# therealadityashankar/hey-buddy

Hardware: AMD Instinct MI355X
Metric: audio clips/sec featurized+trained, 1.5 s @16 kHz, 1/2/4/8 GPU (higher is better)
Workload: dtype f32

## Files before the change

### hey-buddy_amd/csrc/hbk_augment_plan.h

```cpp
#pragma once

#include <algorithm>
#include <cmath>
#include <cstdarg>
#include <cstdint>
#include <cstdio>
#include <numeric>
#include <string>
#include <vector>

namespace hbk {
namespace {

constexpr int kPlanOk = 0, kPlanErrArg = -1, kPlanErrUnsupported = -3;

inline std::string strf(const char* fmt, ...) {
  char buf[512];
  va_list ap;
  va_start(ap, fmt);
  vsnprintf(buf, sizeof(buf), fmt, ap);
  va_end(ap);
  return buf;
}

// ... 79 lines not shown
    return kPlanErrUnsupported;
  }
  return kPlanOk;
}

struct PitchLayout {
  int64_t y = 0;
  int64_t taps = 0;
  int64_t yr = 0;
  int64_t sp = 0;
  int64_t key = 0;
  int64_t ord = 0;
  int64_t gord = 0;
  int64_t total = 0;
};

inline PitchLayout pitch_layout(const PitchGeometry& a, int64_t n) {
  PitchLayout w;
  w.y = 0;
  w.taps = up256(n * a.l1 * 4);
  w.yr = w.taps + up256(int64_t(kPsPhaseMax) * kPsTapMax * 4);
  w.sp = w.yr + up256(n * 8);
  w.key = w.sp + up256(n * 8);
  w.ord = w.key + up256(n * 8);
  w.gord = w.ord + up256(n * 4);
  w.total = w.gord + up256(n * 4);
  return w;
}

struct PitchKnobs {
  bool span = true;
  bool pair = true;
  bool resample_valu = false;
};

struct Grid {
  unsigned x = 1, y = 1, block = 0;
};

struct PitchLaunches {
  bool pair = false;
  int groups = 0;
  Grid taps, span, rank_clips, group, rank_groups, vocoder, resample;
  bool resample_mfma = true;
};

inline PitchLaunches pitch_launches(const PitchGeometry& a, int64_t n, const PitchKnobs& k) {
  PitchLaunches p;
  p.pair = k.span && k.pair;
  p.groups = static_cast<int>((n + kPvClips - 1) / kPvClips);
  p.taps = Grid{unsigned((a.nw * kPsTapMax + 255) / 256), 1, 256};
  p.span = Grid{unsigned((n + 3) / 4), 1, 256};
  p.rank_clips = Grid{unsigned((n + 63) / 64), 1, 1024};
  p.group = Grid{unsigned((p.groups + 255) / 256), 1, 256};
  p.rank_groups = Grid{unsigned((p.groups + 63) / 64), 1, 1024};
  p.vocoder = Grid{unsigned(p.groups), 1, unsigned(128 * kPvClips)};
  const int res_frames = (a.L + a.nw - 1) / a.nw;
  p.resample_mfma = !(k.resample_valu || a.nw > 128);
  p.resample = p.resample_mfma ? Grid{unsigned((res_frames + kRsFrames - 1) / kRsFrames), unsigned(n), 256}
                               : Grid{unsigned((res_frames + kPsResFrames - 1) / kPsResFrames), unsigned(n), 128};
  return p;
}

struct BandStopLayout {
  int64_t sums = 0;
  int64_t taps = 0;
// ... 74 lines not shown
```

### hey-buddy_amd/csrc/hbk_clip_ops.hip

```cpp
#include <algorithm>

#include "hbk_aug_dev.h"

namespace hbk {
namespace {

struct TanhArgs {
  const float* x;
  int64_t x_stride;
  float* out;
  int64_t out_stride;
  int64_t n_clips;
  const float* amount;
  const int32_t* idx;
  int64_t n_entries;
  SrcView view;
};

__device__ __forceinline__ unsigned abs_bits(float v, int s) {
  return s < kT ? (__builtin_bit_cast(unsigned, v) & 0x7FFFFFFFu) : 0xFFFFFFFFu;
}

__global__ void __launch_bounds__(kThreads) __attribute__((amdgpu_waves_per_eu(8)))
tanh_distortion_kernel(TanhArgs a) {
  __shared__ unsigned hist[4096];
  __shared__ float red[32];
  __shared__ unsigned pick[2];
  constexpr int kPer = (kT + kThreads - 1) / kThreads;
  const int64_t n_iter = a.idx ? a.n_entries : a.n_clips;
  for (int64_t e = blockIdx.x; e < n_iter; e += gridDim.x) {
    const int64_t clip = a.idx ? a.idx[e] : e;
    const int tid = opaque_tid();
    const float* x = a.x + clip * a.x_stride;
    float* out = a.out + clip * a.out_stride;
    const float amt = a.amount[clip];
    if (amt != amt) {
      if (out != x) copy_clip(x, out, tid);
      continue;
    }
    float xr[kPer];
    const int pre = a.view.pre ? a.view.pre[clip] : -1, len = a.view.pre ? a.view.len[clip] : 0;
    if (pre >= 0) {
      const int n = min(len, kT);
      const float* row = n > 0 ? a.view.src + clip * a.view.stride : x;
      const int t = opaque_tid();
      const int w0 = __builtin_amdgcn_readfirstlane(t & ~63);
#pragma unroll
      for (int u = 0; u < kPer; ++u) xr[u] = load_placed_wave(row, pre, n, w0 + u * kThreads, t & 63);
    } else {
    const int t = opaque_tid();
#pragma unroll
    for (int u = 0; u < kPer; ++u) {
      const int s = t + u * kThreads;
      xr[u] = s < kT ? *reinterpret_cast<const float*>(reinterpret_cast<const char*>(x) + (static_cast<uint32_t>(s) << 2))
                     : 0.f;
    }
    }
    const double pos = (100.0 - 99.0 * static_cast<double>(amt)) / 100.0 * (kT - 1);
    const int lo = min(max(static_cast<int>(floor(pos)), 0), kT - 1);
    const double frac = pos - lo;
    unsigned prefix = 0, mask = 0, rank = static_cast<unsigned>(lo);
#pragma unroll 1
    for (int p = 0; p < 3; ++p) {
      const int shift = p == 0 ? 19 : (p == 1 ? 9 : 0), bins = p == 0 ? 4096 : (p == 1 ? 1024 : 512);
      const int per_lane = bins >> 6;
      for (int i = tid; i < bins; i += kThreads) hist[i] = 0;
      __syncthreads();
      const int t = opaque_tid();
#pragma unroll
      for (int u = 0; u < kPer; ++u) {
        const unsigned b = abs_bits(xr[u], t + u * kThreads);
        if ((b & mask) == prefix && b != 0xFFFFFFFFu) atomicAdd(&hist[(b >> shift) & (bins - 1)], 1u);
      }
      __syncthreads();
      if (tid < 64) {
        unsigned own = 0;
        for (int i = 0; i < per_lane; ++i) own += hist[per_lane * tid + i];
        unsigned inc = own;
#pragma unroll
        for (int d = 1; d < 64; d <<= 1) {
          const unsigned v = __shfl_up(inc, d, 64);
          if (tid >= d) inc += v;
        }
        const unsigned long long hit = __ballot(inc > rank);
        const int l = __ffsll(static_cast<long long>(hit)) - 1;
        if (tid == l) {
          unsigned r = rank - (inc - own), dsel = per_lane * l;
          for (int i = 0; i < per_lane - 1; ++i) {
            const unsigned h = hist[dsel];
            if (r < h) break;
            r -= h;
            ++dsel;
          }
          pick[0] = dsel;
          pick[1] = r;
        }
      }
      __syncthreads();
      prefix |= pick[0] << shift;
      mask |= static_cast<unsigned>(bins - 1) << shift;
      rank = pick[1];
    }
    float cnt = 0.f, mg = __builtin_inff();
    const int t2 = opaque_tid();
#pragma unroll
    for (int u = 0; u < kPer; ++u) {
// ... 278 lines not shown
```

### hey-buddy_amd/csrc/hbk_pitch.hip

```cpp
#include <atomic>
#include <cstdlib>

#include "hbk_augment_plan.h"
#include "hbk_common.h"

namespace hbk {
namespace {

static_assert(kPsTapMax == HBK_PITCH_SHIFT_MAX_TAPS, "the resampler's tap rows");
static_assert(kPlanOk == HBK_OK && kPlanErrArg == HBK_ERR_ARG && kPlanErrUnsupported == HBK_ERR_UNSUPPORTED,
              "the planner's status values");
#ifndef HBK_PV_ABLATE
#define HBK_PV_ABLATE 0
#endif
#ifndef HBK_PV_F32STATE
#define HBK_PV_F32STATE 0
#endif
#ifndef HBK_PV_RESTART
#if HBK_PV_F32STATE
#define HBK_PV_RESTART 128
#else
#define HBK_PV_RESTART 1024
#endif
#endif
constexpr int kPvRestart = HBK_PV_RESTART;
#if HBK_PV_F32STATE
typedef float pv_t;
#else
typedef double pv_t;
#endif

struct PitchArgs {
  const float* x;
  int64_t x_stride;
  const int32_t* idx;
  int n;
  float* out;
  int64_t out_stride;
  int L, f_in, f_out, l1, orig, nw, width, target;
  double rate;
  float* y;
  float* taps;
  int2* yr;
  int span;
  int2* sp;
  uint64_t* key;
  int32_t* ord;
  int32_t* gord;
};

__device__ __forceinline__ int ps_i0(const PitchArgs& a, int t, float& alpha) {
  const float ts = static_cast<float>(static_cast<double>(t) * a.rate);
  const float fl = floorf(ts);
  alpha = ts - fl;
  return static_cast<int>(fl);
}

struct PvClip {
  float d[kPvRows][8];
  float xs[256];
  float gh[2][kPvGh][8];
  int cnt0;
  int lo, hi;
};
struct PvShared {
  cf tw[256];
  double tw64[256][2];
  float4 wt[3][128];
  PvClip c[kPvClips];
};

__device__ __forceinline__ int pv_g(int b) { return (b & 3) ^ ((b & 4) ? 7 : 0); }

template <int kCtrl>
__device__ __forceinline__ float pv_dpp(float v) {
  return __builtin_bit_cast(float, __builtin_amdgcn_update_dpp(0, __builtin_bit_cast(int, v), kCtrl, 0xF, 0xF, true));
}

template <bool kSwap16>
__device__ __forceinline__ float pv_swap_add(float x, float y) {
  if (kSwap16)
// ... 100 lines not shown
    atomicMax(&C.hi, hi);
  }
}

__device__ __forceinline__ void pv_frames_of(const PitchArgs& a, int lo, int hi, int& tb, int& tl) {
  const int jmax = (a.l1 + kPsPad - 1) / kPsHop;
  tb = 0;
  tl = jmax;
  float al;
  if (lo > hi) {
    tl = -1;
    return;
  }
  if (lo > 2 * kPsPad && a.rate < 2.0) {
    const int fz = (lo - kPsPad) / kPsHop - 1;
    int tg = min(static_cast<int>((fz - 2) / a.rate), a.f_out - 1) & ~(kPvGroup - 1);
    while (tg > 0 && ps_i0(a, tg - 1, al) + 2 > fz) tg -= kPvGroup;
    tb = max(tg, 0);
  }
  if (hi < a.L - 1 - 2 * kPsPad) {
    const int fn = min((hi + kPsPad) / kPsHop, a.f_in - 1);
    int t = max(min(a.f_out - 1, static_cast<int>((fn + 1) / a.rate) + 1), 0);
    while (t > 0 && ps_i0(a, t, al) > fn) --t;
    while (t + 1 < a.f_out && ps_i0(a, t + 1, al) <= fn) ++t;
    tl = min(jmax, t + 36);
  }
}

constexpr int kPsQuant = 360;

__global__ void __launch_bounds__(256) ps_span_kernel(PitchArgs a) {
  const int lane = threadIdx.x & 63, e = blockIdx.x * 4 + (threadIdx.x >> 6);
  if (e >= a.n) return;
  const float* xr = a.x + static_cast<int64_t>(a.idx[e]) * a.x_stride;
  constexpr int kChunk = 64 * 8;
  int lo = INT_MAX, hi = -1;
  for (int p0 = 0; p0 < a.L; p0 += kChunk) {
    float v[8];
#pragma unroll
    for (int j = 0; j < 8; ++j) {
      const int p = p0 + 64 * j + lane;
      v[j] = p < a.L ? xr[p] : 0.f;
    }
#pragma unroll
    for (int j = 0; j < 8; ++j)
      if (v[j] != 0.f) {
        lo = min(lo, p0 + 64 * j + lane);
        hi = max(hi, p0 + 64 * j + lane);
      }
    if (__any(hi >= 0)) break;
  }
  for (int o = 32; o >= 1; o >>= 1) {
    lo = min(lo, __shfl_xor(lo, o, 64));
    hi = max(hi, __shfl_xor(hi, o, 64));
  }
  if (hi >= 0) {
    for (int p1 = a.L; p1 > hi + 1; p1 -= kChunk) {
      float v[8];
      int h = -1;
#pragma unroll
      for (int j = 0; j < 8; ++j) {
        const int p = p1 - kChunk + 64 * j + lane;
        v[j] = (p > hi && p < a.L) ? xr[max(p, 0)] : 0.f;
      }
#pragma unroll
      for (int j = 0; j < 8; ++j)
        if (v[j] != 0.f) h = max(h, p1 - kChunk + 64 * j + lane);
      if (__any(h >= 0)) {
        for (int o = 32; o >= 1; o >>= 1) h = max(h, __shfl_xor(h, o, 64));
        hi = h;
        break;
      }
    }
  }
  if (lane == 0) {
    a.sp[e] = int2{lo, hi};
    const uint64_t q = hi < 0 ? 0 : 1 + static_cast<uint64_t>(hi / kPsQuant), f = hi < 0 ? 0 : static_cast<uint64_t>(lo);
    a.key[e] = (q << 40) | (f << 16) | static_cast<uint64_t>(e);
  }
}

__global__ void __launch_bounds__(1024) ps_rank_kernel(const uint64_t* __restrict__ key, int n,
                                                       int32_t* __restrict__ ord) {
  __shared__ int part[16][64];
  const int lane = threadIdx.x & 63, w = threadIdx.x >> 6, i = blockIdx.x * 64 + lane;
  const uint64_t mine = key[min(i, n - 1)];
  const int per = (n + 15) / 16, j0 = min(w * per, n), j1 = min(j0 + per, n);
  int below = 0;
  for (int jb = j0; jb < j1; jb += 64) {
    const uint64_t kl = jb + lane < j1 ? key[jb + lane] : ~uint64_t(0);
#pragma unroll
    for (int q = 0; q < 64; ++q) {
      const uint32_t hi = __builtin_amdgcn_readlane(static_cast<int>(kl >> 32), q);
      const uint32_t lo = __builtin_amdgcn_readlane(static_cast<int>(kl), q);
      below += ((static_cast<uint64_t>(hi) << 32) | lo) < mine;
    }
// ... 528 lines not shown
#pragma unroll
  for (int ft = 0; ft < kRsFrames / 16; ++ft) {
    rs_f4 acc[2] = {{0.f, 0.f, 0.f, 0.f}, {0.f, 0.f, 0.f, 0.f}};
#pragma unroll
    for (int ks = 0; ks < 5; ++ks) {
      const rs_h8 ah = *reinterpret_cast<const rs_h8*>(&wh[16 * ft + n][32 * ks + 8 * kq]);
      const rs_h8 al = *reinterpret_cast<const rs_h8*>(&wl[16 * ft + n][32 * ks + 8 * kq]);
#pragma unroll
      for (int t = 0; t < 2; ++t) {
        acc[t] = __builtin_amdgcn_mfma_f32_16x16x32_f16(ah, bh[t][ks], acc[t], 0, 0, 0);
        acc[t] = __builtin_amdgcn_mfma_f32_16x16x32_f16(ah, bl[t][ks], acc[t], 0, 0, 0);
        acc[t] = __builtin_amdgcn_mfma_f32_16x16x32_f16(al, bh[t][ks], acc[t], 0, 0, 0);
      }
    }
#pragma unroll
    for (int t = 0; t < 2; ++t) {
      const int ph = 16 * (2 * wave + t) + n;
#pragma unroll
      for (int j = 0; j < 4; ++j) {
        const int i = (f0 + 16 * ft + 4 * kq + j) * a.nw + ph;
        if (ph < a.nw && i < a.L) out[i] = i < a.target ? acc[t][j] * unscale : 0.f;
      }
    }
  }
}

PitchKnobs read_pitch_knobs() {
  PitchKnobs k;
  const char* s = getenv("HBK_PS_SPAN");
  k.span = !(s && s[0] == '0');
  s = getenv("HBK_PS_PAIR");
  k.pair = !(s && s[0] == '0');
  k.resample_valu = getenv("HBK_PS_RESAMPLE_VALU") != nullptr;
  return k;
}

int vocoder_lds_opt_in() {
  constexpr int kDevices = 64;
  static std::atomic<bool> done[kDevices];
  int dev = -1;
  HBK_HIP(hipGetDevice(&dev));
  const bool tracked = dev >= 0 && dev < kDevices;
  if (tracked && done[dev].load(std::memory_order_acquire)) return HBK_OK;
  HBK_HIP(hipFuncSetAttribute(reinterpret_cast<const void*>(ps_vocoder_kernel),
                              hipFuncAttributeMaxDynamicSharedMemorySize, int(sizeof(PvShared))));
  if (tracked) done[dev].store(true, std::memory_order_release);
  return HBK_OK;
}

template <typename... Params, typename... Args>
void launch(void (*kernel)(Params...), const Grid& g, size_t lds, hipStream_t st, Args... args) {
  hipLaunchKernelGGL(kernel, dim3(g.x, g.y), dim3(g.block), lds, st, args...);
}

}

#ifdef HBK_PHASE_TIMING
int pv_phase_take(unsigned long long* out) {
  if (hipMemcpyFromSymbol(out, HIP_SYMBOL(g_pv_phase), sizeof(unsigned long long) * 5) != hipSuccess) return -2;
  unsigned long long z[5] = {};
  (void)hipMemcpyToSymbol(HIP_SYMBOL(g_pv_phase), z, sizeof(z));
  return 0;
}
#endif

}

extern "C" {

int64_t hbk_pitch_shift_workspace_size(int64_t n, int64_t T, int32_t sample_rate, int32_t num, int32_t den) {
  hbk::PitchGeometry g;
  std::string err;
  if (n <= 0 || hbk::pitch_geometry(T, sample_rate, num, den, g, err) != HBK_OK) return 0;
  return hbk::pitch_layout(g, n).total;
}

int hbk_pitch_shift(const float* x, int64_t x_stride, int64_t n, const int32_t* idx, int64_t T, int32_t sample_rate,
                    int32_t num, int32_t den, float* out, int64_t out_stride, void* workspace,
                    int64_t workspace_bytes, void* stream) {
  using namespace hbk;
  if (n < 0) return arg_error("negative n");
  if (n == 0) return HBK_OK;
  if (n > 65535) return arg_error("n > 65535 per call");
  if (!x || !idx || !out || !workspace) return arg_error("NULL pointer");
  PitchGeometry g;
  std::string err;
  const int rc = pitch_geometry(T, sample_rate, num, den, g, err);
  if (rc != HBK_OK) {
    set_error("%s", err.c_str());
    return rc;
  }
  if (x_stride < T || out_stride < T) return arg_error("stride < T");
  const PitchLayout off = pitch_layout(g, n);
  if (workspace_bytes < off.total) return arg_error("workspace too small (hbk_pitch_shift_workspace_size)");
  const PitchKnobs knobs = read_pitch_knobs();
  const PitchLaunches L = pitch_launches(g, n, knobs);
  unsigned char* w = static_cast<unsigned char*>(workspace);
  PitchArgs a{};
  a.x = x;
  a.x_stride = x_stride;
  a.idx = idx;
  a.n = static_cast<int>(n);
  a.out = out;
  a.out_stride = out_stride;
  a.L = g.L, a.f_in = g.f_in, a.f_out = g.f_out, a.l1 = g.l1;
  a.orig = g.orig, a.nw = g.nw, a.width = g.width, a.target = g.target;
  a.rate = g.rate;
  a.y = reinterpret_cast<float*>(w + off.y);
  a.taps = reinterpret_cast<float*>(w + off.taps);
  a.yr = reinterpret_cast<int2*>(w + off.yr);
  a.span = knobs.span ? 1 : 0;
  if (L.pair) {
    a.sp = reinterpret_cast<int2*>(w + off.sp);
    a.key = reinterpret_cast<uint64_t*>(w + off.key);
    a.ord = reinterpret_cast<int32_t*>(w + off.ord);
    a.gord = reinterpret_cast<int32_t*>(w + off.gord);
  }
  const int lds_rc = vocoder_lds_opt_in();
  if (lds_rc != HBK_OK) return lds_rc;
  hipStream_t st = as_stream(stream);
  launch(ps_taps_kernel, L.taps, 0, st, a);
  HBK_LAUNCH_CHECK("ps_taps_kernel");
  if (L.pair) {
    launch(ps_span_kernel, L.span, 0, st, a);
    HBK_LAUNCH_CHECK("ps_span_kernel");
    launch(ps_rank_kernel, L.rank_clips, 0, st, static_cast<const uint64_t*>(a.key), a.n, a.ord);
    HBK_LAUNCH_CHECK("ps_rank_kernel");
    launch(ps_group_kernel, L.group, 0, st, a, L.groups);
    HBK_LAUNCH_CHECK("ps_group_kernel");
    launch(ps_rank_kernel, L.rank_groups, 0, st, static_cast<const uint64_t*>(a.key), L.groups, a.gord);
    HBK_LAUNCH_CHECK("ps_rank_kernel");
  }
  launch(ps_vocoder_kernel, L.vocoder, sizeof(PvShared), st, a);
  HBK_LAUNCH_CHECK("ps_vocoder_kernel");
  launch(L.resample_mfma ? ps_resample_mfma_kernel : ps_resample_kernel, L.resample, 0, st, a);
  HBK_LAUNCH_CHECK(L.resample_mfma ? "ps_resample_mfma_kernel" : "ps_resample_kernel");
  return HBK_OK;
}

}
```

### hey-buddy_amd/heybuddy/_native.py

```python
from __future__ import annotations

import ctypes
import os
import threading
from typing import Optional

import torch

__all__ = ["HBKError", "HBKUnavailable", "lib", "check", "stream_ptr", "require_device",
           "LIB_PATH"]

LIB_PATH = os.environ.get(
    "HBK_LIB",
    os.path.join(os.path.dirname(os.path.dirname(os.path.abspath(__file__))), "lib", "libhbk.so"),
)


class HBKError(RuntimeError):
    """A libhbk.so entry point returned a non-zero status."""


class HBKUnavailable(HBKError):
    """libhbk.so (or a HIP device) is not available: the HIP path cannot run."""

# ... 29 lines not shown
                                     ctypes.POINTER(ctypes.c_double),
                                     ctypes.POINTER(ctypes.c_double),
                                     ctypes.POINTER(ctypes.c_int32)]),
    "hbk_embed_workspace_size": (_c_int, [_vp, _c_int64, ctypes.POINTER(_c_int64)]),
    "hbk_embed_clips": (_c_int, [_vp, _vp, _c_int64, _c_int64, _vp, _vp, _c_int64, _vp]),
    "hbk_embed_split_info": (_c_int, [_vp, ctypes.c_int32, ctypes.POINTER(_c_int64)]),
    "hbk_embed_clips_front": (_c_int, [_vp, _vp, _c_int64, _c_int64, ctypes.c_int32, _vp, _vp, _c_int64, _vp]),
    "hbk_embed_clips_back": (_c_int, [_vp, _vp, _c_int64, ctypes.c_int32, _vp, _vp, _c_int64, _vp]),
    "hbk_embed_windows": (_c_int, [_vp, _vp, _c_int64, _vp, _vp, _c_int64, _vp]),
    "hbk_nan_rows_workspace_size": (_c_int64, [_c_int64]),
    "hbk_nan_rows_fix": (_c_int, [_vp, _c_int64, _c_int64, ctypes.c_uint64, _vp, _c_int64, _vp]),
    "hbk_embed_range_status": (_c_int, [_vp, ctypes.POINTER(ctypes.c_int32), ctypes.c_int32, _vp]),
    "hbk_reverb_plan_create": (_c_int, [_c_int64, ctypes.POINTER(_vp)]),
    "hbk_reverb_plan_destroy": (_c_int, [_vp]),
    "hbk_reverb_spectrum": (_c_int, [_vp, _vp, _c_int64, _c_int64, _vp, _vp]),
    "hbk_augment": (_c_int, [_vp, _vp, _c_int64, _c_int64, _vp, _c_int64, _vp, _vp, _vp, _vp, _vp,
                             _vp, _c_int64, _vp]),
    "hbk_colored_noise": (_c_int, [_vp, _vp, _c_int64, _c_int64, _vp, _c_int64, ctypes.c_uint64, _c_int64, _vp,
                                   _vp, _c_float, _vp, _c_int64, _vp, _c_int64, _vp]),
    "hbk_augment_colored": (_c_int, [_vp, _vp, _c_int64, _c_int64, _vp, _c_int64, _vp, _vp, _vp, _vp, _vp,
                                     _vp, _c_int64, ctypes.c_uint64, _c_int64, _vp, _vp, _c_float, _vp, _c_int64,
                                     _vp, _c_int64, _vp, _c_int64, _vp]),
    "hbk_colored_noise_workspace_size": (_c_int64, [_c_int64, _c_int64]),
    "hbk_colored_noise_ws": (_c_int, [_vp, _vp, _c_int64, _c_int64, _vp, _c_int64, ctypes.c_uint64, _c_int64, _vp,
                                      _vp, _c_float, _vp, _c_int64, _vp, _c_int64, _vp, _c_int64, _vp]),
    "hbk_tanh_distortion": (_c_int, [_vp, _c_int64, _c_int64, _vp, _vp, _c_int64, _vp, _c_int64, _vp]),
    "hbk_band_stop_workspace_size": (_c_int64, [_c_int64, ctypes.c_int32, ctypes.c_int32, _vp]),
    "hbk_band_stop": (_c_int, [_vp, _vp, _c_int64, _c_int64, _vp, _vp, ctypes.c_int32, _vp, _vp, _vp, _vp,
                               ctypes.c_int32, _vp, _vp, _vp, _c_int64, _vp, _c_int64, _vp]),
    "hbk_pitch_shift_workspace_size": (_c_int64, [_c_int64, _c_int64, ctypes.c_int32, ctypes.c_int32,
                                                  ctypes.c_int32]),
    "hbk_pitch_shift": (_c_int, [_vp, _c_int64, _c_int64, _vp, _c_int64, ctypes.c_int32, ctypes.c_int32,
                                 ctypes.c_int32, _vp, _c_int64, _vp, _c_int64, _vp]),
    "hbk_seven_band_eq": (_c_int, [_vp, _c_int64, _c_int64, _vp, _vp, _c_int64, _vp, _c_int64, _vp]),
    "hbk_place_clips": (_c_int, [_vp, _c_int64, _c_int64, _vp, _vp, _vp, _c_int64, _c_int64, _vp]),
    "hbk_place_clips_idx": (_c_int, [_vp, _c_int64, _c_int64, _vp, _vp, _vp, _c_int64, _vp, _c_int64, _c_int64,
                                     _vp]),
    "hbk_seven_band_eq_src": (_c_int, [_vp, _c_int64, _c_int64, _vp, _vp, _c_int64, _vp, _c_int64,
                                       _vp, _c_int64, _vp, _vp, _vp]),
    "hbk_tanh_distortion_src": (_c_int, [_vp, _c_int64, _c_int64, _vp, _vp, _c_int64, _vp, _c_int64,
                                         _vp, _c_int64, _vp, _vp, _vp]),
    "hbk_reverb_plan_set_source": (_c_int, [_vp, _vp, _c_int64, _vp, _vp]),
    "hbk_mlp_set_step_scalars": (_c_int, [_vp, _vp]),
    "hbk_mlp_plan_create": (_c_int, [ctypes.c_int32] * 4 + [ctypes.POINTER(_vp)]),
    "hbk_mlp_plan_create_ex": (_c_int, [ctypes.c_int32] * 6 + [ctypes.POINTER(_vp)]),
    "hbk_mlp_act_forward": (_c_int, [_vp, _c_int64, ctypes.c_int32, ctypes.c_int32, ctypes.c_int32, _vp, _vp]),
    "hbk_mlp_act_backward": (_c_int, [_vp, _vp, _c_int64, ctypes.c_int32, ctypes.c_int32, ctypes.c_int32, _vp,
                                      _vp]),
    "hbk_mlp_plan_create_half": (_c_int, [ctypes.c_int32] * 6 + [_vp, ctypes.POINTER(_vp)]),
    "hbk_mlp_half_layout": (_c_int, [_vp, _vp, ctypes.c_int32]),
    "hbk_mlp_plan_destroy": (_c_int, [_vp]),
    "hbk_mlp_layout": (_c_int, [_vp, ctypes.POINTER(_c_int64), _vp, ctypes.c_int32]),
    "hbk_mlp_workspace_size": (_c_int, [_vp, _c_int64, ctypes.POINTER(_c_int64)]),
    "hbk_mlp_forward": (_c_int, [_vp, _vp, _vp, _c_int64, _vp, _vp, _c_float, ctypes.c_uint64,
                                 _vp, _c_int64, _vp]),
    "hbk_mlp_train_fwd_bwd": (_c_int, [_vp, _vp, _vp, _vp, _c_int64, _c_float, _c_float, _c_float,
                                       _c_float, ctypes.c_uint64, _vp, _vp, _vp, _c_int64, _vp]),
    "hbk_mlp_gate_adam": (_c_int, [_vp, _vp, _vp, _vp, _vp, _vp, _vp, _vp, ctypes.c_int32,
                                   _c_float, _c_float, _c_float, _c_float, _vp]),
    "hbk_mlp_fused_supported": (_c_int, [_vp, ctypes.POINTER(ctypes.c_int32)]),
    "hbk_mlp_step_variant": (_c_int, [_vp, _c_int64, _vp, ctypes.POINTER(ctypes.c_int32)]),
    "hbk_mlp_step_plan_info": (_c_int, [_vp, _c_int64, _vp, ctypes.POINTER(ctypes.c_int32), ctypes.c_int32]),
    "hbk_mlp_step_fwd_bwd": (_c_int, [_vp, _vp, _vp, _c_int64, _vp, _c_int64, _vp, _c_int64, _vp, _c_int64,
                                      _c_int64, _vp, ctypes.c_int32, _vp, _c_int64, _c_float, _c_float,
                                      _c_float, _c_float, ctypes.c_uint64, _vp, _vp, _c_int64, ctypes.c_int32,
                                      _vp, _c_int64, _vp]),
# ... 78 lines not shown
```

### hey-buddy_amd/heybuddy/dataset/augmented.py

```python
from __future__ import annotations

from typing import Any, Dict, Iterator, List, Optional, Sequence

import os
import numpy as np
import torch

from heybuddy.constants import (DEFAULT_AUGMENT_BACKGROUND_NOISE_MAX_SNR_DB,
                                DEFAULT_AUGMENT_BACKGROUND_NOISE_MIN_SNR_DB, DEFAULT_AUGMENT_BAND_STOP_PROB,
                                DEFAULT_AUGMENT_COLORED_NOISE_MAX_F_DECAY,
                                DEFAULT_AUGMENT_COLORED_NOISE_MAX_SNR_DB,
                                DEFAULT_AUGMENT_COLORED_NOISE_MIN_F_DECAY,
                                DEFAULT_AUGMENT_COLORED_NOISE_MIN_SNR_DB, DEFAULT_AUGMENT_COLORED_NOISE_PROB,
                                DEFAULT_AUGMENT_PITCH_SHIFT_PROB, DEFAULT_AUGMENT_PITCH_SHIFT_SEMITONES,
                                DEFAULT_AUGMENT_TANH_DISTORTION_PROB, DEFAULT_AUGMENT_TANH_MAX_DISTORTION,
                                DEFAULT_AUGMENT_TANH_MIN_DISTORTION,
                                DEFAULT_AUGMENT_BACKGROUND_NOISE_PROB, DEFAULT_AUGMENT_GAIN_MAX_DB,
                                DEFAULT_AUGMENT_GAIN_MIN_DB, DEFAULT_AUGMENT_GAIN_PROB,
                                DEFAULT_AUGMENT_REVERB_PROB, DEFAULT_AUGMENT_SEVEN_BAND_GAIN_DB,
                                DEFAULT_AUGMENT_SEVEN_BAND_PROB)
from heybuddy.kernels import ReverbPlan, SourceView, pitch_shift, place_clips, seven_band_eq, tanh_distortion

__all__ = ["AugmentedAudioGenerator", "BatchAugmenter", "SourceOrder", "bandstop_cutoffs", "eq_coefficients",
           "eq_parameters", "hf_shuffle_permutation", "source_plan", "target_length_offset", "target_length_offsets",
# ... 296 lines not shown
            colored = (torch.from_numpy(colored_fd), torch.from_numpy(colored_snr),
                       int(torch.randint(0, 2 ** 62, (1,)).item()))
        pr = {"n": n, "noise_off": torch.from_numpy(noise_off), "spec_idx": torch.from_numpy(spec_idx),
              "snr": snr, "gain": gain, "eq": eq, "tanh": tanh, "bandstop": bandstop, "colored": colored,
              "pitch": [(a, b, _pinned(torch.from_numpy(c))) for a, b, c in getattr(self, "_pitch", [])]}
        pr["route"] = self.routes(pr)
        return pr

    def _colored_fold(self) -> bool:
        return self.sample_rate == 16000 and os.environ.get("HBK_AUG_COLORED_FOLD", "1") != "0"

    def routes(self, pr: Dict[str, Any]) -> np.ndarray:
        n = pr["n"]
        placed_first = np.zeros(n, dtype=bool)
        for _, _, clips in pr.get("pitch") or []:
            placed_first[clips.numpy()] = True
        if pr.get("bandstop") is not None:
            placed_first[pr["bandstop"][0].numpy()] = True
        if pr.get("colored") is not None:
            fd, csnr = pr["colored"][0], pr["colored"][1]
            if self._colored_fold():
                rows = ReverbPlan.colored_fallback_rows(csnr, fd, self.batch_size,
                                                        self.plan.colored_group_path(n, self.batch_size))
                placed_first[rows.numpy()] = True
            else:
                placed_first |= ~torch.isnan(csnr).numpy()
        eq_on = np.zeros(n, dtype=bool)
        if pr.get("eq") is not None:
            eq_on[pr["eq"][1].numpy()] = True
        tanh_on = np.zeros(n, dtype=bool) if pr.get("tanh") is None else ~torch.isnan(pr["tanh"]).numpy()
        return first_touch_routes(eq_on, tanh_on, placed_first)

    def __call__(self, x: torch.Tensor, out: Optional[torch.Tensor] = None,
                 prepared: Optional[Dict[str, Any]] = None, source: Optional[Dict[int, SourceView]] = None
                 ) -> torch.Tensor:
        n = x.shape[0]
        pr = self.prepare(n) if prepared is None else prepared
        if pr["n"] != n:
            raise ValueError(f"prepared for {pr['n']} clips, called with {n}")
        source = source or {}
        if source and (out is None or out.data_ptr() != x.data_ptr()):
            raise ValueError("a source view needs the chain in place (out is x)")
        ev = self._tick("", None)
        if pr["eq"] is not None:
            if out is None:
                out = torch.empty((n, T), dtype=torch.float32, device=x.device)
            if out.data_ptr() != x.data_ptr():
                out.copy_(x[:, :T])
            x = seven_band_eq(out, pr["eq"][0], idx=pr["eq"][1], source=source.get(ROUTE_EQ))
            ev = self._tick("eq", ev)
        if pr["tanh"] is not None:
            x = tanh_distortion(x, pr["tanh"], out=out, source=source.get(ROUTE_TANH))
            out = x
            ev = self._tick("tanh", ev)
        for num, den, clips in pr.get("pitch") or []:
            if out is None:
                out = torch.empty((n, T), dtype=torch.float32, device=x.device)
            x = pitch_shift(x, clips, num, den, out=out, sample_rate=self.sample_rate)
            ev = self._tick("pitch", ev)
        if pr.get("bandstop") is not None:
            if out is None:
                out = x[:, :T].clone()
            elif out.data_ptr() != x.data_ptr():
                out.copy_(x[:, :T])
            x = self.plan.band_stop(out, *pr["bandstop"], out=out)
            ev = self._tick("bandstop", ev)
        colored = None
        if pr["colored"] is not None:
            fd, csnr, seed = pr["colored"]
            if self._colored_fold():
                colored = (fd, csnr, seed, self.batch_size)
            else:
                x = self.plan.colored_noise(x, fd, csnr, seed=seed, out=out, sample_rate=self.sample_rate,
                                            clips_per_noise=self.batch_size)
                out = x
                ev = self._tick("colored", ev)
        y = self.plan.augment(x, self.ring, pr["noise_off"], pr["snr"], self.spectra, pr["spec_idx"],
                              out=out, gain=pr["gain"], colored=colored, source=source.get(ROUTE_AUGMENT))
        self._tick("mix_reverb", ev)
        return y


def source_plan(source_lengths: Sequence[int], num_samples: int, batch_size: int, target_num_samples: int):
    src = np.asarray(source_lengths, dtype=np.int64)
    order = SourceOrder(src.shape[0])
    rows, pres, coins = [], [], []
    for b0 in range(0, int(num_samples), int(batch_size)):
        r = order.take(min(int(batch_size), int(num_samples) - b0))
        rows.append(r)
        pres.append(target_length_offsets(src[r], target_num_samples))
        coins.append(np.random.rand(2))
# ... 165 lines not shown
    def plan_batches(self, lens: Sequence[int]):
        lens = np.asarray(lens, dtype=np.int64)
        pres, coins = [], []
        for b0 in range(0, lens.shape[0], self.batch_size):
            pres.append(target_length_offsets(lens[b0:b0 + self.batch_size], self.target_num_samples))
            coins.append(np.random.rand(2))
        pre = np.concatenate(pres).astype(np.int32) if pres else np.zeros(0, np.int32)
        return pre, np.array(coins, dtype=np.float64).reshape(-1, 2)

    def plan_source(self, source_lengths: Sequence[int], num_samples: int):
        return source_plan(source_lengths, num_samples, self.batch_size, self.target_num_samples)

    def prepare_device(self, clips: torch.Tensor, lengths: Optional[Sequence[int]] = None) -> Dict[str, Any]:
        n = clips.shape[0]
        lens = np.full(n, clips.shape[1], dtype=np.int32) if lengths is None else np.asarray(lengths, np.int32)
        pre, coins = self.plan_batches(lens)
        return {"lens": lens, "pre": pre, "chain": self.augmenter.prepare(n, coins)}

    def augment_device(self, clips: torch.Tensor, lengths: Optional[Sequence[int]] = None,
                       prepared: Optional[Dict[str, Any]] = None) -> torch.Tensor:
        pr = self.prepare_device(clips, lengths) if prepared is None else prepared
        T = self.target_num_samples
        route = pr["chain"].get("route")
        if route is None or not first_touch_enabled() or T != ReverbPlan.T or not clips.shape[1]:
            placed = place_clips(clips, pr["lens"], pr["pre"], T)
            return self.augmenter(placed, out=placed, prepared=pr["chain"])
        n = clips.shape[0]
        lens = np.asarray(pr["lens"], dtype=np.int32).reshape(n)
        pre = np.asarray(pr["pre"], dtype=np.int32).reshape(n)
        if lens.size and (int(lens.min()) < 0 or int(lens.max()) > clips.shape[1] or int(pre.min()) < 0
                          or int((pre + np.minimum(lens, T)).max()) > T):
            raise ValueError("lens / pre must place every clip inside [0, T)")
        routes = (ROUTE_EQ, ROUTE_TANH, ROUTE_AUGMENT)
        host = np.stack([lens, pre] + [np.where(route == r, pre, -1).astype(np.int32) for r in routes])
        dev = _pinned(torch.from_numpy(host)).to(clips.device, non_blocking=True)
        self.placed_rows = np.flatnonzero(route == ROUTE_PLACE).astype(np.int32)
        placed = place_clips(clips, dev[0], dev[1], T, idx=torch.from_numpy(self.placed_rows))
        source = {r: SourceView(clips, dev[0], dev[2 + i]) for i, r in enumerate(routes)}
        return self.augmenter(placed, out=placed, prepared=pr["chain"], source=source)

    def __call__(self, num_samples: int, **kwargs: Any) -> Iterator[Dict[str, Any]]:
        total_batches = int(np.ceil(num_samples / self.batch_size))
        for i in range(total_batches):
            nb = min(self.batch_size, num_samples - i * self.batch_size)
            items = [self.get_next_audio_sample_dict() for _ in range(nb)]
            out = self.execute_augment_batch([it["audio"] for it in items]).cpu().numpy()
            for audio, item in zip(out, items):
                yield {"audio": {"array": audio, "sampling_rate": self.sample_rate},
                       **{k: v for k, v in item.items() if k != "audio"}}


def place_batch_device(src: torch.Tensor, lengths: np.ndarray, pre: np.ndarray, T: int) -> torch.Tensor:
    if not pre.any() and src.shape[1] >= T and (lengths >= T).all():
        return src[:, :T]
    return place_clips(src, lengths, pre, T)
```

### hey-buddy_amd/heybuddy/kernels.py

```python
from __future__ import annotations

import contextlib
import ctypes
import os
import itertools
import threading
from typing import Dict, Optional

import numpy as np
import torch

from heybuddy import _native
from heybuddy._native import check, lib, ptr, stream_ptr

__all__ = ["MelPlan", "mel_frames"]

_plans: Dict[int, object] = {}
_plan_ids = itertools.count(1)
_plans_lock = threading.Lock()


def _register(plan) -> int:
    with _plans_lock:
        pid = next(_plan_ids)
# ... 814 lines not shown


def tanh_distortion(x: torch.Tensor, amount: torch.Tensor, out: torch.Tensor | None = None,
                    source: SourceView | None = None) -> torch.Tensor:
    T = ReverbPlan.T
    dev = _native.require_device(x.device)
    n = x.shape[0]
    if x.dim() != 2 or x.shape[1] < T or x.stride(1) != 1 or x.dtype != torch.float32:
        raise ValueError(f"x must be [n, >= {T}] f32 rows on the device")
    amount = amount.to(dtype=torch.float32).reshape(-1).contiguous()
    if amount.numel() != n:
        raise ValueError("amount must have n entries")
    rows = _active_rows(amount)
    amount = amount.pin_memory().to(dev, non_blocking=True) if amount.device.type == "cpu" else amount.to(dev)
    if out is None:
        out = torch.empty((n, T), dtype=torch.float32, device=dev)
    if rows is not None:
        if out.data_ptr() != x.data_ptr():
            out.copy_(x[:, :T])
            x = out
        if rows.numel() == 0:
            return out
        rows = rows.pin_memory().to(dev, non_blocking=True)
    sv = (None, None, None) if source is None else (source.check(x).src, source.lens, source.pre)
    torch.ops.hbk.tanh_distortion_(x, amount, rows, out, *sv)
    return out


PITCH_SHIFT_CHUNK = 16384
_PS_WS: dict = {}


def pitch_shift(x: torch.Tensor, idx: torch.Tensor, num: int, den: int, out: torch.Tensor | None = None,
                sample_rate: int = 16000) -> torch.Tensor:
    T = ReverbPlan.T
    dev = _native.require_device(x.device)
    if x.dim() != 2 or x.shape[1] < T or x.stride(1) != 1 or x.dtype != torch.float32:
        raise ValueError(f"x must be [n, >= {T}] f32 rows on the device")
    n = x.shape[0]
    if out is None:
        out = torch.empty((n, T), dtype=torch.float32, device=dev)
    if out.data_ptr() != x.data_ptr():
        out.copy_(x[:, :T])
        x = out
    idx = idx.to(dtype=torch.int32).reshape(-1)
    if idx.numel() == 0:
        return out
    if idx.device.type == "cpu":
        if int(idx.min()) < 0 or int(idx.max()) >= n:
            raise ValueError("idx out of range")
        idx = idx.pin_memory().to(dev, non_blocking=True)
    chunk = min(PITCH_SHIFT_CHUNK, idx.numel())
    need = int(lib().hbk_pitch_shift_workspace_size(chunk, T, sample_rate, num, den))
    if need <= 0:
        raise ValueError(f"unsupported pitch shift {num}/{den} at {sample_rate} Hz")
    key = (dev, stream_ptr(dev))
    ws = _PS_WS.get(key)
    if ws is None or ws.numel() < need:
        ws = torch.empty(need, dtype=torch.uint8, device=dev)
        _PS_WS[key] = ws
    for c0 in range(0, idx.numel(), chunk):
        torch.ops.hbk.pitch_shift_(x, idx[c0:c0 + chunk], num, den, sample_rate, out, ws)
    return out


@torch.library.custom_op("hbk::pitch_shift_", mutates_args=("out", "workspace"))
def _pitch_shift_op(x: torch.Tensor, idx: torch.Tensor, num: int, den: int, sample_rate: int, out: torch.Tensor,
                    workspace: torch.Tensor) -> None:
    check(lib().hbk_pitch_shift(ptr(x), x.stride(0), idx.numel(), ptr(idx), ReverbPlan.T, sample_rate, num, den,
                                ptr(out), out.stride(0), ptr(workspace), workspace.numel(), stream_ptr(x.device)),
          "hbk_pitch_shift")


def _view_args(src: torch.Tensor | None, src_len: torch.Tensor | None, src_pre: torch.Tensor | None) -> tuple:
    if src is None:
        return None, 0, None, None
    return ptr(src), src.stride(0), ptr(src_len), ptr(src_pre)


def seven_band_eq(x: torch.Tensor, coef: torch.Tensor, out: torch.Tensor | None = None,
                  idx: torch.Tensor | None = None, source: SourceView | None = None) -> torch.Tensor:
    T = ReverbPlan.T
    dev = _native.require_device(x.device)
    n = x.shape[0]
    if x.dim() != 2 or x.shape[1] < T or x.stride(1) != 1 or x.dtype != torch.float32:
        raise ValueError(f"x must be [n, >= {T}] f32 rows on the device")
    if x.stride(0) % 4 or x.data_ptr() % 16:
        raise ValueError("x rows must be 16-B aligned")

    def to_dev(t: torch.Tensor) -> torch.Tensor:
        return (t if t.is_pinned() else t.pin_memory()).to(dev, non_blocking=True) if t.device.type == "cpu" else t.to(dev)

    m = n if idx is None else int(idx.numel())
    coef = to_dev(coef.to(dtype=torch.float64).reshape(m, 7, 5).contiguous())
    if idx is not None:
        idx = idx.to(dtype=torch.int32).reshape(-1).contiguous()
        if idx.device.type == "cpu" and m and (int(idx.min()) < 0 or int(idx.max()) >= n):
            raise ValueError("idx out of range")
        idx = to_dev(idx)
        if out is None:
            out = x
    elif out is None:
        out = torch.empty((n, T), dtype=torch.float32, device=dev)
    if m:
# ... 332 lines not shown
```

### include/hbk.h

```cpp
#ifndef HBK_H
#define HBK_H

#include <stdint.h>

#ifdef __cplusplus
extern "C" {
#endif

typedef enum {
  HBK_OK = 0,
  HBK_ERR_ARG = -1,
  HBK_ERR_HIP = -2,
  HBK_ERR_UNSUPPORTED = -3
} hbk_status;

const char* hbk_version(void);
const char* hbk_last_error(void);
int hbk_device_count(int* count);
int hbk_stream_create_cu_mask(const uint32_t* cu_mask, int n_words, void** stream);
int hbk_stream_destroy(void* stream);

int hbk_profile_mark(int32_t tag, void* stream);

typedef struct hbk_mel_plan hbk_mel_plan;
// ... 161 lines not shown
int hbk_colored_noise(const hbk_reverb_plan* plan, const float* x, int64_t n_clips, int64_t x_stride,
                      const float* white, int64_t white_stride, uint64_t seed, int64_t clips_per_noise,
                      const float* f_decay, const float* snr_db, float sample_rate, const int32_t* idx,
                      int64_t n_entries, float* out, int64_t out_stride, void* stream);
int64_t hbk_colored_noise_workspace_size(int64_t n_clips, int64_t clips_per_noise);
int hbk_colored_noise_ws(const hbk_reverb_plan* plan, const float* x, int64_t n_clips, int64_t x_stride,
                         const float* white, int64_t white_stride, uint64_t seed, int64_t clips_per_noise,
                         const float* f_decay, const float* snr_db, float sample_rate, const int32_t* idx,
                         int64_t n_entries, float* out, int64_t out_stride, void* workspace, int64_t workspace_bytes,
                         void* stream);

int hbk_augment_colored(const hbk_reverb_plan* plan, const float* x, int64_t n_clips, int64_t x_stride,
                        const float* noise_ring, int64_t ring_len, const int64_t* noise_off,
                        const float* snr_db, const float* spectra, const int32_t* spec_idx,
                        const float* gain, const float* white, int64_t white_stride, uint64_t seed,
                        int64_t clips_per_noise, const float* c_f_decay, const float* c_snr_db,
                        float sample_rate, const int32_t* c_idx, int64_t c_n_entries, float* out,
                        int64_t out_stride, void* workspace, int64_t workspace_bytes, void* stream);

#define HBK_BAND_STOP_CIRCULAR_MAX_HALF 512
#define HBK_BAND_STOP_PARTITION_TAPS 11521
int64_t hbk_band_stop_workspace_size(int64_t n, int32_t n_filters, int32_t n_spectra, void* stream);
int hbk_band_stop(const hbk_reverb_plan* plan, const float* x, int64_t x_stride, int64_t n, const int32_t* idx,
                  const int32_t* filt, int32_t n_filters, const float* f_lo, const float* f_hi,
                  const int32_t* f_half, const int32_t* f_spec0, int32_t n_spectra, const int32_t* s_filt,
                  const int32_t* s_part, float* out, int64_t out_stride, void* workspace, int64_t workspace_bytes,
                  void* stream);

#define HBK_PITCH_SHIFT_MAX_TAPS 144
int64_t hbk_pitch_shift_workspace_size(int64_t n, int64_t T, int32_t sample_rate, int32_t num, int32_t den);
int hbk_pitch_shift(const float* x, int64_t x_stride, int64_t n, const int32_t* idx, int64_t T, int32_t sample_rate,
                    int32_t num, int32_t den, float* out, int64_t out_stride, void* workspace,
                    int64_t workspace_bytes, void* stream);

int hbk_seven_band_eq(const float* x, int64_t n_clips, int64_t x_stride, const double* coef, const int32_t* idx,
                      int64_t n_entries, float* out, int64_t out_stride, void* stream);

int hbk_tanh_distortion(const float* x, int64_t n_clips, int64_t x_stride, const float* amount,
                        const int32_t* idx, int64_t n_entries, float* out, int64_t out_stride, void* stream);

int hbk_place_clips(const float* src, int64_t n_clips, int64_t src_stride, const int32_t* src_len,
                    const int32_t* pre, float* out, int64_t out_stride, int64_t T, void* stream);
int hbk_place_clips_idx(const float* src, int64_t n_clips, int64_t src_stride, const int32_t* src_len,
                        const int32_t* pre, const int32_t* idx, int64_t n_entries, float* out,
                        int64_t out_stride, int64_t T, void* stream);

int hbk_seven_band_eq_src(const float* x, int64_t n_clips, int64_t x_stride, const double* coef,
                          const int32_t* idx, int64_t n_entries, float* out, int64_t out_stride,
                          const float* src, int64_t src_stride, const int32_t* src_len,
                          const int32_t* src_pre, void* stream);
int hbk_tanh_distortion_src(const float* x, int64_t n_clips, int64_t x_stride, const float* amount,
                            const int32_t* idx, int64_t n_entries, float* out, int64_t out_stride,
                            const float* src, int64_t src_stride, const int32_t* src_len,
                            const int32_t* src_pre, void* stream);
int hbk_reverb_plan_set_source(hbk_reverb_plan* plan, const float* src, int64_t src_stride,
                               const int32_t* src_len, const int32_t* src_pre);

#ifdef __cplusplus
}
#endif

#endif
```

Baseline: 1.138 million.

## Bound pitch-shift span scan by known clip placement; ballot-count zeros in tanh histogram

The pitch-shift span kernel now receives each row's placement offset and length from the host, so it scans only the placed clip region for nonzero extent instead of the whole row. The tanh distortion radix-select counts exact-zero samples once per wave with a ballot and adds them to bin 0 in a single atomic, rather than having every zero sample do its own LDS atomic. Both changes cut memory reads and LDS atomic contention. The span change adds a new API entry and extra plumbing, and relies on rows outside the placed span being zero.

```diff
diff --git a/hey-buddy_amd/csrc/hbk_augment_plan.h b/hey-buddy_amd/csrc/hbk_augment_plan.h
--- a/hey-buddy_amd/csrc/hbk_augment_plan.h
+++ b/hey-buddy_amd/csrc/hbk_augment_plan.h
@@ -135,6 +135,7 @@
   bool span = true;
   bool pair = true;
   bool resample_valu = false;
+  bool span_known = true;
 };
 
 struct Grid {
diff --git a/hey-buddy_amd/csrc/hbk_clip_ops.hip b/hey-buddy_amd/csrc/hbk_clip_ops.hip
--- a/hey-buddy_amd/csrc/hbk_clip_ops.hip
+++ b/hey-buddy_amd/csrc/hbk_clip_ops.hip
@@ -21,6 +21,9 @@
   return s < kT ? (__builtin_bit_cast(unsigned, v) & 0x7FFFFFFFu) : 0xFFFFFFFFu;
 }
 
+#ifndef HBK_TANH_ZERO_BALLOT
+#define HBK_TANH_ZERO_BALLOT 1
+#endif
 __global__ void __launch_bounds__(kThreads) __attribute__((amdgpu_waves_per_eu(8)))
 tanh_distortion_kernel(TanhArgs a) {
   __shared__ unsigned hist[4096];
@@ -60,6 +63,17 @@
     const int lo = min(max(static_cast<int>(floor(pos)), 0), kT - 1);
     const double frac = pos - lo;
     unsigned prefix = 0, mask = 0, rank = static_cast<unsigned>(lo);
+    int zeros = 0;
+#if HBK_TANH_ZERO_BALLOT
+    {
+      const int t = opaque_tid();
+#pragma unroll
+      for (int u = 0; u < kPer; ++u) {
+        zeros += __popcll(__ballot(abs_bits(xr[u], t + u * kThreads) == 0));
+        asm volatile("" : "+s"(zeros));
+      }
+    }
+#endif
 #pragma unroll 1
     for (int p = 0; p < 3; ++p) {
       const int shift = p == 0 ? 19 : (p == 1 ? 9 : 0), bins = p == 0 ? 4096 : (p == 1 ? 1024 : 512);
@@ -70,8 +84,13 @@
 #pragma unroll
       for (int u = 0; u < kPer; ++u) {
         const unsigned b = abs_bits(xr[u], t + u * kThreads);
+#if HBK_TANH_ZERO_BALLOT
+        if ((b & mask) == prefix && b - 1u < 0xFFFFFFFEu) atomicAdd(&hist[(b >> shift) & (bins - 1)], 1u);
+#else
         if ((b & mask) == prefix && b != 0xFFFFFFFFu) atomicAdd(&hist[(b >> shift) & (bins - 1)], 1u);
-      }
+#endif
+      }
+      if (HBK_TANH_ZERO_BALLOT && prefix == 0 && zeros && (t & 63) == 0) atomicAdd(&hist[0], unsigned(zeros));
       __syncthreads();
       if (tid < 64) {
         unsigned own = 0;
diff --git a/hey-buddy_amd/csrc/hbk_pitch.hip b/hey-buddy_amd/csrc/hbk_pitch.hip
--- a/hey-buddy_amd/csrc/hbk_pitch.hip
+++ b/hey-buddy_amd/csrc/hbk_pitch.hip
@@ -47,6 +47,8 @@
   uint64_t* key;
   int32_t* ord;
   int32_t* gord;
+  const int32_t* kpre;
+  const int32_t* klen;
 };
 
 __device__ __forceinline__ int ps_i0(const PitchArgs& a, int t, float& alpha) {
@@ -213,15 +215,23 @@
 __global__ void __launch_bounds__(256) ps_span_kernel(PitchArgs a) {
   const int lane = threadIdx.x & 63, e = blockIdx.x * 4 + (threadIdx.x >> 6);
   if (e >= a.n) return;
-  const float* xr = a.x + static_cast<int64_t>(a.idx[e]) * a.x_stride;
+  const int row = a.idx[e];
+  int b0 = 0, b1 = a.L;
+  if (a.kpre) {
+    const int pre = a.kpre[row];
+    if (pre >= 0) b0 = min(pre, a.L), b1 = pre + min(a.klen[row], a.L - pre);
+    b0 = __builtin_amdgcn_readfirstlane(b0);
+    b1 = __builtin_amdgcn_readfirstlane(b1);
+  }
+  const float* xr = a.x + static_cast<int64_t>(row) * a.x_stride;
   constexpr int kChunk = 64 * 8;
   int lo = INT_MAX, hi = -1;
-  for (int p0 = 0; p0 < a.L; p0 += kChunk) {
+  for (int p0 = b0; p0 < b1; p0 += kChunk) {
     float v[8];
 #pragma unroll
     for (int j = 0; j < 8; ++j) {
       const int p = p0 + 64 * j + lane;
-      v[j] = p < a.L ? xr[p] : 0.f;
+      v[j] = p < b1 ? xr[p] : 0.f;
     }
 #pragma unroll
     for (int j = 0; j < 8; ++j)
@@ -236,13 +246,13 @@
     hi = max(hi, __shfl_xor(hi, o, 64));
   }
   if (hi >= 0) {
-    for (int p1 = a.L; p1 > hi + 1; p1 -= kChunk) {
+    for (int p1 = b1; p1 > hi + 1; p1 -= kChunk) {
       float v[8];
       int h = -1;
 #pragma unroll
       for (int j = 0; j < 8; ++j) {
         const int p = p1 - kChunk + 64 * j + lane;
-        v[j] = (p > hi && p < a.L) ? xr[max(p, 0)] : 0.f;
+        v[j] = (p > hi && p < b1) ? xr[max(p, 0)] : 0.f;
       }
 #pragma unroll
       for (int j = 0; j < 8; ++j)
@@ -837,6 +847,8 @@
   s = getenv("HBK_PS_PAIR");
   k.pair = !(s && s[0] == '0');
   k.resample_valu = getenv("HBK_PS_RESAMPLE_VALU") != nullptr;
+  s = getenv("HBK_PS_SPAN_KNOWN");
+  k.span_known = !(s && s[0] == '0');
   return k;
 }
 
@@ -883,11 +895,20 @@
 int hbk_pitch_shift(const float* x, int64_t x_stride, int64_t n, const int32_t* idx, int64_t T, int32_t sample_rate,
                     int32_t num, int32_t den, float* out, int64_t out_stride, void* workspace,
                     int64_t workspace_bytes, void* stream) {
+  return hbk_pitch_shift_span(x, x_stride, n, idx, T, sample_rate, num, den, out, out_stride, workspace,
+                              workspace_bytes, nullptr, nullptr, stream);
+}
+
+int hbk_pitch_shift_span(const float* x, int64_t x_stride, int64_t n, const int32_t* idx, int64_t T,
+                         int32_t sample_rate, int32_t num, int32_t den, float* out, int64_t out_stride,
+                         void* workspace, int64_t workspace_bytes, const int32_t* span_pre,
+                         const int32_t* span_len, void* stream) {
   using namespace hbk;
   if (n < 0) return arg_error("negative n");
   if (n == 0) return HBK_OK;
   if (n > 65535) return arg_error("n > 65535 per call");
   if (!x || !idx || !out || !workspace) return arg_error("NULL pointer");
+  if ((span_pre == nullptr) != (span_len == nullptr)) return arg_error("span_pre and span_len come together");
   PitchGeometry g;
   std::string err;
   const int rc = pitch_geometry(T, sample_rate, num, den, g, err);
@@ -920,6 +941,7 @@
     a.key = reinterpret_cast<uint64_t*>(w + off.key);
     a.ord = reinterpret_cast<int32_t*>(w + off.ord);
     a.gord = reinterpret_cast<int32_t*>(w + off.gord);
+    if (knobs.span_known) a.kpre = span_pre, a.klen = span_len;
   }
   const int lds_rc = vocoder_lds_opt_in();
   if (lds_rc != HBK_OK) return lds_rc;
diff --git a/hey-buddy_amd/heybuddy/_native.py b/hey-buddy_amd/heybuddy/_native.py
--- a/hey-buddy_amd/heybuddy/_native.py
+++ b/hey-buddy_amd/heybuddy/_native.py
@@ -85,6 +85,8 @@
                                                   ctypes.c_int32]),
     "hbk_pitch_shift": (_c_int, [_vp, _c_int64, _c_int64, _vp, _c_int64, ctypes.c_int32, ctypes.c_int32,
                                  ctypes.c_int32, _vp, _c_int64, _vp, _c_int64, _vp]),
+    "hbk_pitch_shift_span": (_c_int, [_vp, _c_int64, _c_int64, _vp, _c_int64, ctypes.c_int32, ctypes.c_int32,
+                                      ctypes.c_int32, _vp, _c_int64, _vp, _c_int64, _vp, _vp, _vp]),
     "hbk_seven_band_eq": (_c_int, [_vp, _c_int64, _c_int64, _vp, _vp, _c_int64, _vp, _c_int64, _vp]),
     "hbk_place_clips": (_c_int, [_vp, _c_int64, _c_int64, _vp, _vp, _vp, _c_int64, _c_int64, _vp]),
     "hbk_place_clips_idx": (_c_int, [_vp, _c_int64, _c_int64, _vp, _vp, _vp, _c_int64, _vp, _c_int64, _c_int64,
diff --git a/hey-buddy_amd/heybuddy/dataset/augmented.py b/hey-buddy_amd/heybuddy/dataset/augmented.py
--- a/hey-buddy_amd/heybuddy/dataset/augmented.py
+++ b/hey-buddy_amd/heybuddy/dataset/augmented.py
@@ -352,8 +352,8 @@
         return first_touch_routes(eq_on, tanh_on, placed_first)
 
     def __call__(self, x: torch.Tensor, out: Optional[torch.Tensor] = None,
-                 prepared: Optional[Dict[str, Any]] = None, source: Optional[Dict[int, SourceView]] = None
-                 ) -> torch.Tensor:
+                 prepared: Optional[Dict[str, Any]] = None, source: Optional[Dict[int, SourceView]] = None,
+                 span: Optional[tuple] = None) -> torch.Tensor:
         n = x.shape[0]
         pr = self.prepare(n) if prepared is None else prepared
         if pr["n"] != n:
@@ -376,7 +376,7 @@
         for num, den, clips in pr.get("pitch") or []:
             if out is None:
                 out = torch.empty((n, T), dtype=torch.float32, device=x.device)
-            x = pitch_shift(x, clips, num, den, out=out, sample_rate=self.sample_rate)
+            x = pitch_shift(x, clips, num, den, out=out, sample_rate=self.sample_rate, span=span)
             ev = self._tick("pitch", ev)
         if pr.get("bandstop") is not None:
             if out is None:
@@ -608,12 +608,14 @@
                           or int((pre + np.minimum(lens, T)).max()) > T):
             raise ValueError("lens / pre must place every clip inside [0, T)")
         routes = (ROUTE_EQ, ROUTE_TANH, ROUTE_AUGMENT)
-        host = np.stack([lens, pre] + [np.where(route == r, pre, -1).astype(np.int32) for r in routes])
+        host = np.stack([lens, pre] + [np.where(route == r, pre, -1).astype(np.int32) for r in routes]
+                        + [np.where(route != ROUTE_EQ, pre, -1).astype(np.int32)])
         dev = _pinned(torch.from_numpy(host)).to(clips.device, non_blocking=True)
         self.placed_rows = np.flatnonzero(route == ROUTE_PLACE).astype(np.int32)
         placed = place_clips(clips, dev[0], dev[1], T, idx=torch.from_numpy(self.placed_rows))
         source = {r: SourceView(clips, dev[0], dev[2 + i]) for i, r in enumerate(routes)}
-        return self.augmenter(placed, out=placed, prepared=pr["chain"], source=source)
+        span = (dev[5], dev[0]) if pr["chain"].get("pitch") else None
+        return self.augmenter(placed, out=placed, prepared=pr["chain"], source=source, span=span)
 
     def __call__(self, num_samples: int, **kwargs: Any) -> Iterator[Dict[str, Any]]:
         total_batches = int(np.ceil(num_samples / self.batch_size))
diff --git a/hey-buddy_amd/heybuddy/kernels.py b/hey-buddy_amd/heybuddy/kernels.py
--- a/hey-buddy_amd/heybuddy/kernels.py
+++ b/hey-buddy_amd/heybuddy/kernels.py
@@ -870,12 +870,16 @@
 
 
 def pitch_shift(x: torch.Tensor, idx: torch.Tensor, num: int, den: int, out: torch.Tensor | None = None,
-                sample_rate: int = 16000) -> torch.Tensor:
+                sample_rate: int = 16000, span: tuple | None = None) -> torch.Tensor:
     T = ReverbPlan.T
     dev = _native.require_device(x.device)
     if x.dim() != 2 or x.shape[1] < T or x.stride(1) != 1 or x.dtype != torch.float32:
         raise ValueError(f"x must be [n, >= {T}] f32 rows on the device")
     n = x.shape[0]
+    for t in span or ():
+        if t.dtype != torch.int32 or t.shape != (n,) or t.device != dev or not t.is_contiguous():
+            raise ValueError("span must be (pre, len), int32 [n] on x's device")
+    span_pre, span_len = span or (None, None)
     if out is None:
         out = torch.empty((n, T), dtype=torch.float32, device=dev)
     if out.data_ptr() != x.data_ptr():
@@ -898,16 +902,19 @@
         ws = torch.empty(need, dtype=torch.uint8, device=dev)
         _PS_WS[key] = ws
     for c0 in range(0, idx.numel(), chunk):
-        torch.ops.hbk.pitch_shift_(x, idx[c0:c0 + chunk], num, den, sample_rate, out, ws)
+        torch.ops.hbk.pitch_shift_(x, idx[c0:c0 + chunk], num, den, sample_rate, out, ws, span_pre, span_len)
     return out
 
 
 @torch.library.custom_op("hbk::pitch_shift_", mutates_args=("out", "workspace"))
 def _pitch_shift_op(x: torch.Tensor, idx: torch.Tensor, num: int, den: int, sample_rate: int, out: torch.Tensor,
-                    workspace: torch.Tensor) -> None:
-    check(lib().hbk_pitch_shift(ptr(x), x.stride(0), idx.numel(), ptr(idx), ReverbPlan.T, sample_rate, num, den,
-                                ptr(out), out.stride(0), ptr(workspace), workspace.numel(), stream_ptr(x.device)),
-          "hbk_pitch_shift")
+                    workspace: torch.Tensor, span_pre: torch.Tensor | None = None,
+                    span_len: torch.Tensor | None = None) -> None:
+    check(lib().hbk_pitch_shift_span(ptr(x), x.stride(0), idx.numel(), ptr(idx), ReverbPlan.T, sample_rate, num, den,
+                                     ptr(out), out.stride(0), ptr(workspace), workspace.numel(),
+                                     None if span_pre is None else ptr(span_pre),
+                                     None if span_len is None else ptr(span_len), stream_ptr(x.device)),
+          "hbk_pitch_shift_span")
 
 
 def _view_args(src: torch.Tensor | None, src_len: torch.Tensor | None, src_pre: torch.Tensor | None) -> tuple:
diff --git a/include/hbk.h b/include/hbk.h
--- a/include/hbk.h
+++ b/include/hbk.h
@@ -217,6 +217,10 @@
 int hbk_pitch_shift(const float* x, int64_t x_stride, int64_t n, const int32_t* idx, int64_t T, int32_t sample_rate,
                     int32_t num, int32_t den, float* out, int64_t out_stride, void* workspace,
                     int64_t workspace_bytes, void* stream);
+int hbk_pitch_shift_span(const float* x, int64_t x_stride, int64_t n, const int32_t* idx, int64_t T,
+                         int32_t sample_rate, int32_t num, int32_t den, float* out, int64_t out_stride,
+                         void* workspace, int64_t workspace_bytes, const int32_t* span_pre,
+                         const int32_t* span_len, void* stream);
 
 int hbk_seven_band_eq(const float* x, int64_t n_clips, int64_t x_stride, const double* coef, const int32_t* idx,
                       int64_t n_entries, float* out, int64_t out_stride, void* stream);
```

Result: no change. 1.149 million, median of 6 (+1.0%).
